# WxuanYuan/diffusynth

Measured on AMD Instinct MI355X. Metric: denoising-steps/sec (batch x T) on 256x64 latents, higher is better.
Workload: dtype bf16x3; 1 GPU; BASELINE configs[2]: DiffSynthSampler.sample() wall-clock, production ConditionedUnet (random init, torch.manual_seed(0)), bf16x3 (fp32 tensors, dense convolutions as 3 bf16 MFMA terms with fp32 accumulation: meets 1e-3 vs the fp32 reference), batch 64/GPU, latent (4,256,64), text condition, CFG=6.0 (U-Net batch 128 per step), 33-step respaced ddpm schedule, Philox noise on device; global_batch=64, parallelism=batch-shard x1, weights replicated

## Files before the change

### diffusynth_amd/csrc/dwconv_gn.hip

```cpp
#include <type_traits>

#include "common.hpp"

namespace {

constexpr int DW_TH = 4;
constexpr int DW_BLOCK = 256;

struct DwSrc { const char* base; int Cs, cc, Hs, Ws, oh, ow, buf; };
template <int ES>
__device__ __forceinline__ DwSrc dw_src(const ds_dwconv_params& p, int b, int c0) {
    if (c0 < p.C0) return {reinterpret_cast<const char*>(p.src0) + (size_t)b * p.H * p.W * p.C0 * ES, p.C0, c0, p.H, p.W, 0, 0, DS_BX_SRC0};
    return {reinterpret_cast<const char*>(p.src1) + (size_t)b * p.H1 * p.W1 * p.C1 * ES, p.C1, c0 - p.C0, p.H1, p.W1, p.off_h1, p.off_w1, DS_BX_SRC1};
}

template <int SR, int V, typename LoadRow>
__device__ __forceinline__ void dw_tap_column(float (&acc)[SR][V], const float* wcol, int pitch, LoadRow load_row) {
    float wv[7][V];
#pragma unroll
    for (int dh = 0; dh < 7; ++dh)
#pragma unroll
        for (int v = 0; v < V; v += 4) {
            const f32x4 t4 = *reinterpret_cast<const f32x4*>(wcol + dh * pitch + v);
            wv[dh][v] = t4[0]; wv[dh][v + 1] = t4[1]; wv[dh][v + 2] = t4[2]; wv[dh][v + 3] = t4[3];
        }
#pragma unroll
    for (int r = 0; r < SR + 6; ++r) {
        float x[V];
        load_row(r, x);
#pragma unroll
        for (int dh = 0; dh < 7; ++dh) {
            const int o = r - dh;
            if (o >= 0 && o < SR) {
#pragma unroll
                for (int v = 0; v < V; ++v) acc[o][v] = fmaf(x[v], wv[dh][v], acc[o][v]);
            }
        }
    }
}

template <typename T>
__device__ __forceinline__ float2 dw_store_row(const ds_dwconv_params& p, bool split, int b, int h, int w, int C, int c, const float* a, float2 s) {
    if (split) {
        bf16* o2 = reinterpret_cast<bf16*>(p.out) + ((size_t)b * p.H * p.W + (size_t)(h * p.W + w)) * (2 * C) + c;
        uint2 hi, lo;
        ds_split2(a[0], a[1], hi.x, lo.x);
        ds_split2(a[2], a[3], hi.y, lo.y);
        DS_ST(bf16x4, o2, DS_BX_OUT, __builtin_bit_cast(bf16x4, hi));
        DS_ST(bf16x4, o2 + C, DS_BX_OUT, __builtin_bit_cast(bf16x4, lo));
    } else {
        T* outp = reinterpret_cast<T*>(p.out) + (size_t)b * p.H * p.W * C;
        vec16_store<T>(outp + ((size_t)(h * p.W + w) * C + c), a, DS_BX_OUT);
    }
#pragma unroll
    for (int v = 0; v < Vec16<T>::N; ++v) {
        s.x += a[v];
        s.y += a[v] * a[v];
    }
    return s;
}

template <typename T>
__global__ __launch_bounds__(DW_BLOCK) void dwconv7_kernel(const ds_dwconv_params p, int nstrip, int CV) {
    constexpr int V = Vec16<T>::N;
    __shared__ float red[2 * (DW_BLOCK / 64)];
    const int C = p.C0 + p.C1;
    const int b = blockIdx.y;
    const long gid = (long)blockIdx.x * DW_BLOCK + threadIdx.x;
    const long total = (long)nstrip * p.W * CV;
    float2 st = {0.f, 0.f};
    if (gid < total) {
        const int cv = gid % CV;
        const int w = (gid / CV) % p.W;
        const int strip = gid / ((long)CV * p.W);
        const int h0 = strip * DW_TH;
        const int c = cv * V;
        const DwSrc s = dw_src<sizeof(T)>(p, b, c);
        const T* base = reinterpret_cast<const T*>(s.base);
        float acc[DW_TH][V];
        float init[V];
#pragma unroll
        for (int v = 0; v < V; ++v) {
            init[v] = p.bias[c + v];
            if (p.tbias) init[v] += p.tbias[(size_t)b * p.tb_stride + c + v];
        }
#pragma unroll
        for (int t = 0; t < DW_TH; ++t)
#pragma unroll
            for (int v = 0; v < V; ++v) acc[t][v] = init[v];

        for (int dw = 0; dw < 7; ++dw) {
            const int wi = w + dw - 3 - s.ow;
            if ((unsigned)wi >= (unsigned)s.Ws) continue;
            float col[DW_TH + 6][V];
#pragma unroll
            for (int r = 0; r < DW_TH + 6; ++r) {
                const int hi = h0 + r - 3 - s.oh;
                if ((unsigned)hi < (unsigned)s.Hs) {
                    vec16_load<T>(base + ((size_t)(hi * s.Ws + wi) * s.Cs + s.cc), col[r], s.buf);
                } else {
#pragma unroll
                    for (int v = 0; v < V; ++v) col[r][v] = 0.f;
                }
            }
#pragma unroll
            for (int dh = 0; dh < 7; ++dh) {
                float wv[V];
                const float* wp = p.wt + (size_t)(dh * 7 + dw) * C + c;
#pragma unroll
                for (int v = 0; v < V; v += 4) {
                    f32x4 t4 = DS_LD(f32x4, wp + v, DS_BX_W);
                    wv[v] = t4[0]; wv[v + 1] = t4[1]; wv[v + 2] = t4[2]; wv[v + 3] = t4[3];
                }
#pragma unroll
                for (int t = 0; t < DW_TH; ++t)
#pragma unroll
                    for (int v = 0; v < V; ++v) acc[t][v] = fmaf(col[t + dh][v], wv[v], acc[t][v]);
            }
        }
#pragma unroll
        for (int t = 0; t < DW_TH; ++t)
            if (h0 + t < p.H) st = dw_store_row<T>(p, false, b, h0 + t, w, C, c, acc[t], st);
    }
    if (p.stats_part) block_stats_write(st.x, st.y, red, p.stats_part + ((size_t)b * gridDim.x + blockIdx.x) * 2);
}

constexpr int LT_SR = 8;
constexpr int LT_NT = 2048 / LT_SR;
template <int TWL, int NV>
struct LT {
    static constexpr int W = 1 << TWL, H = (2048 / NV) >> TWL, HC = W + 6, HR = H + 6, NPX = HC * HR;
};
static int lt_twl(int W, int nv) { return W <= 8 ? 3 : ((W <= 16 || nv == 8) ? 4 : 5); }

template <typename T, int TWL, int LT_NV>
__global__ __launch_bounds__(LT_NT) void dwconv7_lds_kernel(const ds_dwconv_params p, int tiles_w, int tiles_hw, int ncblk) {
    constexpr int LT_W = LT<TWL, LT_NV>::W, LT_H = LT<TWL, LT_NV>::H, LT_HC = LT<TWL, LT_NV>::HC, LT_NPX = LT<TWL, LT_NV>::NPX;
    static_assert(LT_NV * LT_W * (LT_H / LT_SR) == LT_NT && LT_H % LT_SR == 0, "thread map");
    constexpr int V = Vec16<T>::N;
    constexpr int CB = LT_NV * V;
    extern __shared__ __attribute__((aligned(16))) char dsm[];
    uint4* xs = reinterpret_cast<uint4*>(dsm);
    float* wsm = reinterpret_cast<float*>(dsm + (size_t)LT_NPX * LT_NV * 16);
    float* red = wsm + 49 * CB;
    const int tid = threadIdx.x;
    const int wid = blockIdx.x + gridDim.x * blockIdx.y;
    const int cblk = wid % ncblk, tile = (wid / ncblk) % tiles_hw, b = wid / (tiles_hw * ncblk);
    const int bix = tile * ncblk + cblk;
    const int th = tile / tiles_w, tw = tile - th * tiles_w;
    const int h0 = th * LT_H, w0 = tw * LT_W, c0 = cblk * CB;
    const int C = p.C0 + p.C1;
    const DwSrc s = dw_src<sizeof(T)>(p, b, c0);
    const T* base = reinterpret_cast<const T*>(s.base);
#if DS_BOUNDS
    for (int slot = tid; slot < LT_NPX * LT_NV; slot += LT_NT) {
        const int px = slot / LT_NV, v = slot - px * LT_NV;
        const int hr = px / LT_HC, hc = px - hr * LT_HC;
        const int hi = h0 + hr - 3 - s.oh, wi = w0 + hc - 3 - s.ow;
        uint4 val = make_uint4(0, 0, 0, 0);
        if ((unsigned)hi < (unsigned)s.Hs && (unsigned)wi < (unsigned)s.Ws)
            val = DS_LD(uint4, base + ((size_t)(hi * s.Ws + wi) * s.Cs + s.cc + v * V), s.buf);
        xs[slot] = val;
    }
    for (int i = tid; i < 49 * CB; i += LT_NT) wsm[i] = DS_LD(float, p.wt + (size_t)(i / CB) * C + c0 + (i % CB), DS_BX_W);
#else
    {
        constexpr int SLOTS = LT_NPX * LT_NV, ITS = (SLOTS + LT_NT - 1) / LT_NT;
        const __amdgpu_buffer_rsrc_t rs = __builtin_amdgcn_make_buffer_rsrc(const_cast<T*>(base), (short)0, (int)((size_t)s.Hs * s.Ws * s.Cs * sizeof(T)), 0x00020000);
        const __amdgpu_buffer_rsrc_t rs_w = __builtin_amdgcn_make_buffer_rsrc(const_cast<float*>(p.wt), (short)0, 49 * C * 4, 0x00020000);
        u32x4 hv[ITS];
#pragma unroll
        for (int it = 0; it < ITS; ++it) {
            const int slot = tid + it * LT_NT;
            const int px = slot / LT_NV, v = slot - px * LT_NV;
            const int hr = px / LT_HC, hc = px - hr * LT_HC;
            const int hi = h0 + hr - 3 - s.oh, wi = w0 + hc - 3 - s.ow;
            const unsigned bad = (unsigned)(slot >= SLOTS) | (unsigned)((unsigned)hi >= (unsigned)s.Hs) | (unsigned)((unsigned)wi >= (unsigned)s.Ws);
            const unsigned off = (unsigned)((hi * s.Ws + wi) * s.Cs + s.cc + v * V) * (unsigned)sizeof(T);
            hv[it] = __builtin_amdgcn_raw_buffer_load_b128(rs, (int)((off & 0x7fffffffu) | (bad << 31)), 0, 0);
        }
        constexpr int WP = 49 * CB / 4, WIT = (WP + LT_NT - 1) / LT_NT;
        asm volatile("" : "+v"(hv[ITS - 1]));
        u32x4 wv4[WIT];
#pragma unroll
        for (int k = 0; k < WIT; ++k) {
            const int wp = tid + k * LT_NT, wtap = wp / (CB / 4), wj = wp - wtap * (CB / 4);
            wv4[k] = __builtin_amdgcn_raw_buffer_load_b128(rs_w, (int)((unsigned)((wtap * C + c0 + 4 * wj) * 4) | ((unsigned)(wp >= WP) << 31)), 0, 0);
        }
#pragma unroll
        for (int it = 0; it < ITS; ++it) {
            const int slot = tid + it * LT_NT;
            if (it + 1 < ITS || slot < SLOTS) *reinterpret_cast<u32x4*>(xs + slot) = hv[it];
        }
#pragma unroll
        for (int k = 0; k < WIT; ++k)
            if (tid + k * LT_NT < WP) *reinterpret_cast<u32x4*>(wsm + 4 * (tid + k * LT_NT)) = wv4[k];
    }
#endif
    const int cv = tid % LT_NV, wl = (tid / LT_NV) % LT_W, strip = tid / (LT_NV * LT_W);
    const int c = c0 + cv * V;
    float acc[LT_SR][V];
    {
        float init[V];
#if DS_BOUNDS
#pragma unroll
        for (int v = 0; v < V; ++v) {
            init[v] = p.bias[c + v];
            if (p.tbias) init[v] += p.tbias[(size_t)b * p.tb_stride + c + v];
        }
#else
        const __amdgpu_buffer_rsrc_t rs_b = __builtin_amdgcn_make_buffer_rsrc(const_cast<float*>(p.bias), (short)0, C * 4, 0x00020000);
        const __amdgpu_buffer_rsrc_t rs_t = __builtin_amdgcn_make_buffer_rsrc(const_cast<float*>(p.tbias ? p.tbias + (size_t)b * p.tb_stride : p.bias),
                                                                               (short)0, p.tbias ? C * 4 : 0, 0x00020000);
#pragma unroll
        for (int v = 0; v < V; v += 4) {
            const u32x4 b4 = __builtin_amdgcn_raw_buffer_load_b128(rs_b, (c + v) * 4, 0, 0), t4 = __builtin_amdgcn_raw_buffer_load_b128(rs_t, (c + v) * 4, 0, 0);
#pragma unroll
            for (int j = 0; j < 4; ++j) init[v + j] = __uint_as_float(b4[j]) + __uint_as_float(t4[j]);
        }
#endif
        __syncthreads();
#pragma unroll
        for (int o = 0; o < LT_SR; ++o)
#pragma unroll
            for (int v = 0; v < V; ++v) acc[o][v] = init[v];
    }
#pragma unroll 1
    for (int dw = 0; dw < 7; ++dw)
        dw_tap_column<LT_SR, V>(acc, wsm + dw * CB + cv * V, 7 * CB, [&](int r, float* x) {
            Vec16<T>::load(reinterpret_cast<const T*>(xs + ((strip * LT_SR + r) * LT_HC + wl + dw) * LT_NV + cv), x);
        });
    float2 st = {0.f, 0.f};
    const int w = w0 + wl;
#pragma unroll
    for (int o = 0; o < LT_SR; ++o) {
        const int h = h0 + strip * LT_SR + o;
        if (h < p.H && w < p.W) st = dw_store_row<T>(p, sizeof(T) == 4 && p.out_split, b, h, w, C, c, acc[o], st);
    }
    if (p.stats_part) block_stats_write(st.x, st.y, red, p.stats_part + ((size_t)b * gridDim.x + bix) * 2);
}

constexpr int ST_W = 16, ST_R = 16, ST_HC = ST_W + 6, ST_HR = ST_R + 6, ST_NT = 256;
constexpr int ST_ROWB = ST_HC * 8 * 16;
constexpr int ST_XS = ST_HR * ST_ROWB;
constexpr int ST_LDS = ST_XS + 49 * 32 * 4 + 64;

__global__ __launch_bounds__(ST_NT, 2) void dwconv7_strip_kernel(const ds_dwconv_params p, int strips_w, int ncblk, int hparts, int rows_per_part) {
    extern __shared__ __attribute__((aligned(16))) char dsm[];
    char* const xs = dsm;
    float* const wsm = reinterpret_cast<float*>(dsm + ST_XS);
    float* const red = wsm + 49 * 32;
    const int tid = threadIdx.x;
    const int nwg = gridDim.x;
    int wid = blockIdx.x;
    if ((nwg & 7) == 0) wid = (wid & 7) * (nwg >> 3) + (wid >> 3);
    const int cblk = wid % ncblk, sw = (wid / ncblk) % strips_w, hp = (wid / (strips_w * ncblk)) % hparts, b = wid / (strips_w * ncblk * hparts);
    const int bix = (hp * strips_w + sw) * ncblk + cblk;
    const int w0 = sw * ST_W, c0 = cblk * 32;
    const int hbeg = hp * rows_per_part, hend = min(p.H, hbeg + rows_per_part);
    const int ntile = (hend - hbeg + ST_R - 1) / ST_R;
    const int C = p.C0 + p.C1;
    const DwSrc s = dw_src<4>(p, b, c0);
    const int hc = tid >> 3, sv = tid & 7;
    const bool stager = hc < ST_HC;
    const int wi = w0 + hc - 3 - s.ow;
    const bool col_ok = stager && (unsigned)wi < (unsigned)s.Ws;
    const unsigned colbyte = (unsigned)((wi * s.Cs + s.cc + sv * 4) * 4);
    const unsigned rowpitch = (unsigned)(s.Ws * s.Cs * 4);
#if !DS_BOUNDS
    const __amdgpu_buffer_rsrc_t rs = __builtin_amdgcn_make_buffer_rsrc(const_cast<char*>(s.base), (short)0, (int)((size_t)s.Hs * s.Ws * s.Cs * 4), 0x00020000);
#endif
    auto load_rows = [&](u32x4* dst, int row0, auto nc) {
        constexpr int n = decltype(nc)::value;
#pragma unroll
        for (int it = 0; it < n; ++it) {
            const int hi = row0 + it - s.oh;
            const unsigned bad = (unsigned)(!col_ok) | (unsigned)((unsigned)hi >= (unsigned)s.Hs);
#if DS_BOUNDS
            dst[it] = u32x4{0u, 0u, 0u, 0u};
            if (!bad) dst[it] = DS_LD(u32x4, s.base + (size_t)hi * rowpitch + colbyte, s.buf);
#else
            const unsigned off = (unsigned)hi * rowpitch + colbyte;
            dst[it] = __builtin_amdgcn_raw_buffer_load_b128(rs, (int)((off & 0x7fffffffu) | (bad << 31)), 0, 0);
#endif
        }
    };
    auto store_rows = [&](const u32x4* src, int slot0, auto nc) {
        constexpr int n = decltype(nc)::value;
#pragma unroll
        for (int it = 0; it < n; ++it) {
            int sl = slot0 + it;
            sl = sl >= ST_HR ? sl - ST_HR : sl;
            *reinterpret_cast<u32x4*>(xs + sl * ST_ROWB + tid * 16) = src[it];
        }
    };
    auto lds_barrier = [&]() {
        asm volatile("s_waitcnt lgkmcnt(0)" ::: "memory");
        __builtin_amdgcn_s_barrier();
        asm volatile("" ::: "memory");
    };
    using N6 = std::integral_constant<int, 6>;
    using N16 = std::integral_constant<int, ST_R>;

    u32x4 hv[ST_R];
    u32x4 h6[6];
    if (stager) {
        load_rows(h6, hbeg - 3, N6{});
        load_rows(hv, hbeg + 3, N16{});
    }
    {
        constexpr int WP = 49 * 32 / 4, WIT = (WP + ST_NT - 1) / ST_NT;
#pragma unroll
        for (int k = 0; k < WIT; ++k) {
            const int wp = tid + k * ST_NT, wtap = wp >> 3, wj = wp & 7;
            if (wp < WP) *reinterpret_cast<f32x4*>(wsm + 4 * wp) = DS_LD(f32x4, p.wt + (size_t)wtap * C + c0 + 4 * wj, DS_BX_W);
        }
    }
    const int cv = tid & 7, wl = (tid >> 3) & 15, strip = tid >> 7;
    const int c = c0 + cv * 4;
    float init[4];
    {
        const f32x4 b4 = DS_LD(f32x4, p.bias + c, DS_BX_BIAS);
        f32x4 t4 = {0.f, 0.f, 0.f, 0.f};
        if (p.tbias) t4 = DS_LD(f32x4, p.tbias + (size_t)b * p.tb_stride + c, DS_BX_AUX1);
#pragma unroll
        for (int j = 0; j < 4; ++j) init[j] = b4[j] + t4[j];
    }
    if (stager) {
        store_rows(h6, 0, N6{});
        store_rows(hv, 6, N16{});
    }
    lds_barrier();

    float2 st = {0.f, 0.f};
    int rbase = 0;
    const int w = w0 + wl;
    const int colb = wl * 128 + cv * 16;
#pragma unroll 1
    for (int t = 0; t < ntile; ++t) {
        const int htop = hbeg + t * ST_R;
        const bool more = t + 1 < ntile;
        if (more && stager) load_rows(hv, htop + ST_R + 3, N16{});
        int roff[LT_SR + 6];
#pragma unroll
        for (int r = 0; r < LT_SR + 6; ++r) {
            int sl = rbase + strip * LT_SR + r;
            sl = sl >= ST_HR ? sl - ST_HR : sl;
            sl = sl >= ST_HR ? sl - ST_HR : sl;
            roff[r] = sl * ST_ROWB + colb;
        }
        float acc[LT_SR][4];
#pragma unroll
        for (int o = 0; o < LT_SR; ++o)
#pragma unroll
            for (int v = 0; v < 4; ++v) acc[o][v] = init[v];
#pragma unroll 1
        for (int dw = 0; dw < 7; ++dw)
            dw_tap_column<LT_SR, 4>(acc, wsm + dw * 32 + cv * 4, 7 * 32, [&](int r, float* x) {
                Vec16<float>::load(reinterpret_cast<const float*>(xs + roff[r] + dw * 128), x);
            });
        lds_barrier();
        if (more) {
            int ws = rbase + ST_R + 6;
            ws = ws >= ST_HR ? ws - ST_HR : ws;
            ws = ws >= ST_HR ? ws - ST_HR : ws;
            if (stager) store_rows(hv, ws, N16{});
            rbase = rbase + ST_R >= ST_HR ? rbase + ST_R - ST_HR : rbase + ST_R;
        }
#pragma unroll
        for (int o = 0; o < LT_SR; ++o) {
            const int h = htop + strip * LT_SR + o;
            if (h < hend && w < p.W) st = dw_store_row<float>(p, p.out_split, b, h, w, C, c, acc[o], st);
        }
        if (more) lds_barrier();
    }
    __syncthreads();
    if (p.stats_part) block_stats_write(st.x, st.y, red, p.stats_part + ((size_t)b * (hparts * strips_w * ncblk) + bix) * 2);
}

constexpr int MF_CB = 32;
template <bool TALL> struct M2 {
    static constexpr int W = TALL ? 16 : 32, H = TALL ? 32 : 16;
    static constexpr int HR = H + 6;
    static constexpr int HC = TALL ? 24 : 40;
    static constexpr int PLANE = HR * HC, SKEW = 32;
    static constexpr int BLK2 = TALL ? 16 * HC : 16;
    static constexpr int PBYTES = (MF_CB * PLANE + 3 * SKEW) * 2;
    static constexpr int OFF_O = 2 * PBYTES, OBYTES = H * W * MF_CB * 2, OFF_RED = OFF_O + OBYTES, LDS = OFF_RED + 64;
    static constexpr int SLOTS = HR * (HC / 4) * 4;
    static_assert(LDS <= 160 * 1024, "one block per CU");
};

struct Dw2Geo { int tiles_w, tiles, ncblk, tpc, nchunk, total; };
typedef __amdgpu_buffer_rsrc_t dw_rsrc_t;
__device__ __forceinline__ u32x4 dw_buf_ld16(dw_rsrc_t rs, const char* base, unsigned voff, int bounds_buf) {
#if DS_BOUNDS
    if (voff >= 0x80000000u || !ds_bx_ok(base + voff, bounds_buf, 16)) return u32x4{0u, 0u, 0u, 0u};
#endif
    (void)base; (void)bounds_buf;
    return __builtin_amdgcn_raw_buffer_load_b128(rs, (int)voff, 0, 0);
}

template <int NW, bool TALL>
__global__ __launch_bounds__(NW * 64, 1) void dwconv7_mfma2_kernel(const ds_dwconv_params p, const Dw2Geo g) {
    using G = M2<TALL>;
    constexpr int M2_W = G::W, M2_H = G::H, M2_HC = G::HC, M2_PLANE = G::PLANE, M2_SKEW = G::SKEW, M2_PBYTES = G::PBYTES, M2_OFF_O = G::OFF_O,
                  M2_OFF_RED = G::OFF_RED, M2_SLOTS = G::SLOTS;
    constexpr int NT = NW * 64, CPW = MF_CB / NW, SIT = (M2_SLOTS + NT - 1) / NT, OIT = M2_H * M2_W * 4 / NT;
    extern __shared__ __attribute__((aligned(16))) char dsm[];
    float* red = reinterpret_cast<float*>(dsm + M2_OFF_RED);
    const int tid = threadIdx.x, lane = tid & 63, wave = tid >> 6;
    const int NB = gridDim.x;
    int lid = blockIdx.x;
    if (NB % 8 == 0) lid = (blockIdx.x & 7) * (NB >> 3) + (blockIdx.x >> 3);
    if (lid >= g.total) return;
    const int nmy = (g.total - lid + NB - 1) / NB;
    const int nt = nmy * g.tpc - ((lid + (nmy - 1) * NB) / g.ncblk == g.nchunk - 1 ? g.nchunk * g.tpc - p.B * g.tiles : 0);
    const int C = p.C0 + p.C1;
    const bf16* wexp = reinterpret_cast<const bf16*>(p.wexp);

    struct Tile { dw_rsrc_t rs; int c, j, tile, th, tw, b, c0, h0, w0; DwSrc s; };
    auto set_sample = [&](Tile& t) {
        t.s = dw_src<2>(p, t.b, t.c0);
        t.rs = __builtin_amdgcn_make_buffer_rsrc(const_cast<char*>(t.s.base), (short)0, t.s.Hs * t.s.Ws * t.s.Cs * 2, 0x00020000);
    };
    auto start_chunk = [&](int c) {
        Tile t;
        t.c = c;
        t.j = 0;
        const int cblk = c % g.ncblk, item = (c / g.ncblk) * g.tpc;
        t.b = item / g.tiles;
        t.tile = item - t.b * g.tiles;
        t.th = t.tile / g.tiles_w;
        t.tw = t.tile - t.th * g.tiles_w;
        t.h0 = t.th * M2_H;
        t.w0 = t.tw * M2_W;
        t.c0 = cblk * MF_CB;
        set_sample(t);
        return t;
    };
    auto next_tile = [&](Tile t) {
        if (t.j + 1 == g.tpc) return start_chunk(t.c + NB);
        ++t.j;
        if (++t.tile == g.tiles) {
            t.tile = 0; t.th = 0; t.tw = 0;
            ++t.b;
            set_sample(t);
        } else if (++t.tw == g.tiles_w) { t.tw = 0; ++t.th; }
        t.h0 = t.th * M2_H;
        t.w0 = t.tw * M2_W;
        return t;
    };

    int s_hr[SIT], s_hc[SIT], s_lds[SIT];
    bool s_ok[SIT];
    const int sv = tid & 3;
#pragma unroll
    for (int it = 0; it < SIT; ++it) {
        const int slot = tid + it * NT, qd = slot >> 2;
        s_ok[it] = slot < M2_SLOTS;
        s_hr[it] = qd / (M2_HC / 4);
        s_hc[it] = (qd - s_hr[it] * (M2_HC / 4)) * 4;
        s_lds[it] = ((sv * 8) * M2_PLANE + sv * M2_SKEW + s_hr[it] * M2_HC + s_hc[it]) * 2;
    }
    u32x4 fv[SIT][4];
    auto issue_halo = [&](const Tile& t) {
#pragma unroll
        for (int it = 0; it < SIT; ++it) {
            const int hi = t.h0 + s_hr[it] - 3 - t.s.oh, wi = t.w0 + s_hc[it] - 3 - t.s.ow;
            const unsigned badr = (unsigned)(!s_ok[it]) | (unsigned)((unsigned)hi >= (unsigned)t.s.Hs);
            const unsigned o = (unsigned)((hi * t.s.Ws + wi) * t.s.Cs + t.s.cc + sv * 8) * 2u;
#pragma unroll
            for (int e = 0; e < 4; ++e) {
                const unsigned bad = badr | (unsigned)((unsigned)(wi + e) >= (unsigned)t.s.Ws);
                fv[it][e] = dw_buf_ld16(t.rs, t.s.base, ((o + (unsigned)(e * t.s.Cs) * 2u) & 0x0fffffffu) | (bad << 31), t.s.buf);
            }
        }
    };
    auto fill_planes = [&](char* pl) {
#pragma unroll
        for (int it = 0; it < SIT; ++it) {
            if (s_ok[it]) {
                char* dst = pl + s_lds[it];
#pragma unroll
                for (int j = 0; j < 4; ++j) {
                    const unsigned a = fv[it][0][j], b2 = fv[it][1][j], c2 = fv[it][2][j], d = fv[it][3][j];
                    typedef unsigned u32x2_t __attribute__((ext_vector_type(2)));
                    *reinterpret_cast<u32x2_t*>(dst + (2 * j) * (M2_PLANE * 2)) =
                        u32x2_t{__builtin_amdgcn_perm(b2, a, 0x05040100u), __builtin_amdgcn_perm(d, c2, 0x05040100u)};
                    *reinterpret_cast<u32x2_t*>(dst + (2 * j + 1) * (M2_PLANE * 2)) =
                        u32x2_t{__builtin_amdgcn_perm(b2, a, 0x07060302u), __builtin_amdgcn_perm(d, c2, 0x07060302u)};
                }
            }
        }
    };

    const int m = lane & 15, kq = lane >> 4;
    int aoff[6];
#pragma unroll
    for (int ks = 0; ks < 6; ++ks) {
        const int dh = 4 * (ks & 1) + kq, wg = ks >> 1;
        aoff[ks] = (m + (dh > 6 ? 6 : dh)) * M2_HC + 8 * wg;
    }
    bf16x8 wv[CPW][6];
    float addv[CPW];
    auto load_addv = [&](const Tile& t) {
        const int cb = t.c0 + wave * CPW;
#pragma unroll
        for (int k = 0; k < CPW; ++k) {
            addv[k] = DS_LD(float, p.bias + cb + k, DS_BX_BIAS);
            if (p.tbias) addv[k] += DS_LD(float, p.tbias + (size_t)t.b * p.tb_stride + cb + k, DS_BX_AUX1);
        }
    };
    auto load_chunk_consts = [&](const Tile& t) {
        const int cb = t.c0 + wave * CPW;
#pragma unroll
        for (int ci = 0; ci < CPW; ++ci) {
            const bf16* we = wexp + ((size_t)(cb + ci) * 6 * 64 + lane) * 8;
#pragma unroll
            for (int ks = 0; ks < 6; ++ks) wv[ci][ks] = DS_LD(bf16x8, we + ks * 64 * 8, DS_BX_AUX0);
        }
        load_addv(t);
    };

    Tile cur = start_chunk(lid);
    issue_halo(cur);
    load_chunk_consts(cur);
    fill_planes(dsm);
    __syncthreads();
    float s1 = 0.f, s2 = 0.f;
    char* const ot = dsm + M2_OFF_O;
    auto tile_body = [&](const int u, auto more_t) {
        constexpr bool more = decltype(more_t)::value;
        char* const pl = dsm + (u & 1) * M2_PBYTES;
        Tile nxt = cur;
        if constexpr (more) {
            nxt = next_tile(cur);
            issue_halo(nxt);
        }
        float outv[2][4][CPW];
#pragma unroll
        for (int ci = 0; ci < CPW; ++ci) {
            const int cl = wave * CPW + ci;
            const bf16* plane = reinterpret_cast<const bf16*>(pl) + cl * M2_PLANE + (cl >> 3) * M2_SKEW;
            f32x4 acc0 = {0.f, 0.f, 0.f, 0.f}, acc1 = {0.f, 0.f, 0.f, 0.f};
#pragma unroll
            for (int ks = 0; ks < 6; ++ks) {
                const bf16x8 a0 = *reinterpret_cast<const bf16x8*>(plane + aoff[ks]);
                const bf16x8 a1 = *reinterpret_cast<const bf16x8*>(plane + aoff[ks] + G::BLK2);
                acc0 = __builtin_amdgcn_mfma_f32_16x16x32_bf16(a0, wv[ci][ks], acc0, 0, 0, 0);
                acc1 = __builtin_amdgcn_mfma_f32_16x16x32_bf16(a1, wv[ci][ks], acc1, 0, 0, 0);
            }
#pragma unroll
            for (int r = 0; r < 4; ++r) {
                outv[0][r][ci] = acc0[r] + addv[ci];
                outv[1][r][ci] = acc1[r] + addv[ci];
            }
        }
#pragma unroll
        for (int wb = 0; wb < 2; ++wb)
#pragma unroll
            for (int r = 0; r < 4; ++r)
                if (cur.h0 + (TALL ? 16 * wb : 0) + kq * 4 + r < p.H && cur.w0 + (TALL ? 0 : 16 * wb) + m < p.W) {
#pragma unroll
                    for (int v = 0; v < CPW; ++v) {
                        s1 += outv[wb][r][v];
                        s2 = fmaf(outv[wb][r][v], outv[wb][r][v], s2);
                    }
                }
#pragma unroll
        for (int wb = 0; wb < 2; ++wb)
#pragma unroll
            for (int r = 0; r < 4; ++r) {
                typedef __bf16 bf16xc_t __attribute__((ext_vector_type(CPW)));
                bf16xc_t pk;
#pragma unroll
                for (int v = 0; v < CPW; ++v) pk[v] = (bf16)outv[wb][r][v];
                const int col = (TALL ? 0 : 16 * wb) + m, row = (TALL ? 16 * wb : 0) + kq * 4 + r, cbyte = wave * CPW * 2;
                *reinterpret_cast<bf16xc_t*>(ot + (row * M2_W + col) * 64 + (((cbyte >> 4) ^ ((col >> 1) & 3)) * 16) + (cbyte & 15)) = pk;
            }
        __syncthreads();
        const bool chunk_end = cur.j + 1 == g.tpc, sample_end = chunk_end || cur.tile + 1 == g.tiles;
        if (sample_end && p.stats_part) {
            const int nps = g.tiles >= g.tpc ? g.tiles / g.tpc : 1, kk = g.tiles >= g.tpc ? cur.tile / g.tpc : 0;
            block_stats_write(s1, s2, red, p.stats_part + ((size_t)cur.b * (nps * g.ncblk) + kk * g.ncblk + cur.c0 / MF_CB) * 2);
            s1 = 0.f;
            s2 = 0.f;
        }
        if constexpr (more) {
            if (chunk_end || sample_end) {
                if (chunk_end) load_chunk_consts(nxt);
                else load_addv(nxt);
#pragma unroll
                for (int ci = 0; ci < CPW; ++ci)
#pragma unroll
                    for (int ks = 0; ks < 6; ++ks) asm volatile("" : "+v"(wv[ci][ks]));
#pragma unroll
                for (int ci = 0; ci < CPW; ++ci) asm volatile("" : "+v"(addv[ci]));
            }
            fill_planes(dsm + ((u + 1) & 1) * M2_PBYTES);
        }
        {
            bf16* outp = reinterpret_cast<bf16*>(p.out) + (size_t)cur.b * p.H * p.W * C;
#pragma unroll
            for (int k = 0; k < OIT; ++k) {
                const int piece = tid + k * NT, px = piece >> 2, q = piece & 3;
                const int col = px % M2_W, h = cur.h0 + px / M2_W, w = cur.w0 + col;
                if (h < p.H && w < p.W) {
                    const u32x4 v = *reinterpret_cast<const u32x4*>(ot + px * 64 + ((q ^ ((col >> 1) & 3)) * 16));
                    DS_ST(u32x4, outp + ((size_t)(h * p.W + w) * C + cur.c0 + q * 8), DS_BX_OUT, v);
                }
            }
        }
        __syncthreads();
        cur = nxt;
    };
    for (int u = 0; u + 1 < nt; ++u) tile_body(u, std::true_type{});
    tile_body(nt - 1, std::false_type{});
}

static int dw_batch(const ds_dwconv_params* p) { return p->batch_hint > 0 ? p->batch_hint : p->B; }

static bool dw_tall(const ds_dwconv_params* p) { return p->W <= 16; }
static Dw2Geo dw2_geo(const ds_dwconv_params* p) {
    const int tw = dw_tall(p) ? 16 : 32, th = dw_tall(p) ? 32 : 16;
    Dw2Geo g;
    g.tiles_w = (p->W + tw - 1) / tw;
    g.tiles = g.tiles_w * ((p->H + th - 1) / th);
    g.ncblk = (p->C0 + p->C1) / MF_CB;
    g.tpc = 1;
    for (int d = 2; d <= 8; ++d)
        if ((g.tiles % d == 0 || (d % g.tiles == 0 && dw_batch(p) % (d / g.tiles) == 0 && g.ncblk <= 256)) && (long long)dw_batch(p) * g.tiles / d * g.ncblk >= 512) g.tpc = d;
    g.nchunk = (p->B * g.tiles + g.tpc - 1) / g.tpc;
    g.total = g.nchunk * g.ncblk;
    return g;
}

__global__ void pack_dw_mfma_kernel(const float* w, int C, bf16* dst) {
    const long i = (long)blockIdx.x * blockDim.x + threadIdx.x;
    if (i >= (long)C * 6 * 64 * 8) return;
    const int j = i & 7, lane = (i >> 3) & 63, ks = (i >> 9) % 6, c = i / (6 * 64 * 8);
    const int n = lane & 15, kq = lane >> 4;
    const int dh = 4 * (ks & 1) + kq, wg = ks >> 1, wp = 8 * wg + j, dw = wp - n;
    float v = 0.f;
    if (dh < 7 && dw >= 0 && dw < 7) v = w[(size_t)c * 49 + dh * 7 + dw];
    dst[i] = (bf16)v;
}

__global__ void pack_dw_kernel(const float* w, int C, float* dst) {
    const int i = blockIdx.x * blockDim.x + threadIdx.x;
    if (i < 49 * C) dst[i] = w[(size_t)(i % C) * 49 + i / C];
}

__global__ void gn_finalize_kernel(const float* part, int parts, double count, float eps, float* ab) {
    __shared__ double r1[256], r2[256];
    const int b = blockIdx.x;
    double a = 0.0, q = 0.0;
    for (int i = threadIdx.x; i < parts; i += blockDim.x) {
        a += (double)part[((size_t)b * parts + i) * 2];
        q += (double)part[((size_t)b * parts + i) * 2 + 1];
    }
    r1[threadIdx.x] = a;
    r2[threadIdx.x] = q;
// ... 601 lines not shown
```

Baseline: 721.8 denoising-steps/s.

## Software-pipeline depthwise 7x7 stencil with fully unrolled prefetched LDS loads

Replaces the per-column tap loop (runtime loop over dw, with weights loaded per column) with a fully unrolled 49-tap stencil that issues LDS weight and input-row loads a few taps ahead (DW_AHEAD=3). Scheduling barriers and empty asm constraints pin the ordering so the LDS load latency overlaps the FMAs. Input rows are loaded once per column as raw vectors and converted in place. This raises code size and register pressure, which could lower occupancy or cause spills under the kernel's launch bounds.

```diff
diff --git a/diffusynth_amd/csrc/dwconv_gn.hip b/diffusynth_amd/csrc/dwconv_gn.hip
--- a/diffusynth_amd/csrc/dwconv_gn.hip
+++ b/diffusynth_amd/csrc/dwconv_gn.hip
@@ -14,29 +14,60 @@
     return {reinterpret_cast<const char*>(p.src1) + (size_t)b * p.H1 * p.W1 * p.C1 * ES, p.C1, c0 - p.C0, p.H1, p.W1, p.off_h1, p.off_w1, DS_BX_SRC1};
 }
 
-template <int SR, int V, typename LoadRow>
-__device__ __forceinline__ void dw_tap_column(float (&acc)[SR][V], const float* wcol, int pitch, LoadRow load_row) {
-    float wv[7][V];
-#pragma unroll
-    for (int dh = 0; dh < 7; ++dh)
-#pragma unroll
-        for (int v = 0; v < V; v += 4) {
-            const f32x4 t4 = *reinterpret_cast<const f32x4*>(wcol + dh * pitch + v);
-            wv[dh][v] = t4[0]; wv[dh][v + 1] = t4[1]; wv[dh][v + 2] = t4[2]; wv[dh][v + 3] = t4[3];
-        }
-#pragma unroll
-    for (int r = 0; r < SR + 6; ++r) {
-        float x[V];
-        load_row(r, x);
-#pragma unroll
-        for (int dh = 0; dh < 7; ++dh) {
-            const int o = r - dh;
-            if (o >= 0 && o < SR) {
-#pragma unroll
-                for (int v = 0; v < V; ++v) acc[o][v] = fmaf(x[v], wv[dh][v], acc[o][v]);
-            }
-        }
-    }
+#ifndef DW_AHEAD
+#define DW_AHEAD 3
+#endif
+template <int G, int N, typename F>
+__device__ __forceinline__ void dw_static_for(F f) {
+    if constexpr (G < N) {
+        f(std::integral_constant<int, G>{});
+        dw_static_for<G + 1, N>(f);
+    }
+}
+template <typename T, int SR, int AHEAD, typename WAt, typename RowAt>
+__device__ __forceinline__ void dw_stencil(float (&acc)[SR][Vec16<T>::N], WAt w_at, RowAt row_at) {
+    constexpr int V = Vec16<T>::N;
+    f32x4 wr[49][V / 4];
+    u32x4 xr[7][SR + 6];
+    auto request = [&](auto gc) {
+        constexpr int g = decltype(gc)::value, dw = g / 7, dh = g % 7;
+#pragma unroll
+        for (int v = 0; v < V / 4; ++v) wr[g][v] = *reinterpret_cast<const f32x4*>(w_at(dw, dh) + 4 * v);
+#pragma unroll
+        for (int r = (dh ? dh + SR - 1 : 0); r < dh + SR; ++r) xr[dw][r] = *reinterpret_cast<const u32x4*>(row_at(dw, r));
+    };
+    dw_static_for<0, AHEAD>(request);
+    dw_static_for<0, 49>([&](auto gc) {
+        constexpr int g = decltype(gc)::value, dw = g / 7, dh = g % 7;
+        if constexpr (g + AHEAD < 49) request(std::integral_constant<int, g + AHEAD>{});
+        asm volatile("" : : : "memory");
+        __builtin_amdgcn_sched_barrier(0);
+#pragma unroll
+        for (int o = 0; o < SR; ++o) {
+            float x[V];
+            if constexpr (V == 4) {
+#pragma unroll
+                for (int v = 0; v < V; ++v) x[v] = __uint_as_float(xr[dw][o + dh][v]);
+            } else {
+                const bf16x8 b8 = __builtin_bit_cast(bf16x8, xr[dw][o + dh]);
+#pragma unroll
+                for (int v = 0; v < V; ++v) x[v] = (float)b8[v];
+            }
+#pragma unroll
+            for (int v = 0; v < V; ++v) acc[o][v] = fmaf(x[v], wr[g][v >> 2][v & 3], acc[o][v]);
+        }
+        if constexpr (g + 1 < 49) {
+#pragma unroll
+            for (int o = 0; o < SR; ++o)
+#pragma unroll
+                for (int v = 0; v < V; v += 4) {
+                    f32x4 a4 = {acc[o][v], acc[o][v + 1], acc[o][v + 2], acc[o][v + 3]};
+                    asm volatile("" : "+v"(a4) : : "memory");
+                    acc[o][v] = a4[0]; acc[o][v + 1] = a4[1]; acc[o][v + 2] = a4[2]; acc[o][v + 3] = a4[3];
+                }
+        }
+        __builtin_amdgcn_sched_barrier(0);
+    });
 }
 
 template <typename T>
@@ -225,11 +256,8 @@
 #pragma unroll
             for (int v = 0; v < V; ++v) acc[o][v] = init[v];
     }
-#pragma unroll 1
-    for (int dw = 0; dw < 7; ++dw)
-        dw_tap_column<LT_SR, V>(acc, wsm + dw * CB + cv * V, 7 * CB, [&](int r, float* x) {
-            Vec16<T>::load(reinterpret_cast<const T*>(xs + ((strip * LT_SR + r) * LT_HC + wl + dw) * LT_NV + cv), x);
-        });
+    dw_stencil<T, LT_SR, DW_AHEAD>(acc, [&](int dw, int dh) { return wsm + (dh * 7 + dw) * CB + cv * V; },
+                                   [&](int dw, int r) { return xs + ((strip * LT_SR + r) * LT_HC + wl + dw) * LT_NV + cv; });
     float2 st = {0.f, 0.f};
     const int w = w0 + wl;
 #pragma unroll
@@ -348,17 +376,15 @@
             sl = sl >= ST_HR ? sl - ST_HR : sl;
             sl = sl >= ST_HR ? sl - ST_HR : sl;
             roff[r] = sl * ST_ROWB + colb;
+            asm volatile("" : "+v"(roff[r]));
         }
         float acc[LT_SR][4];
 #pragma unroll
         for (int o = 0; o < LT_SR; ++o)
 #pragma unroll
             for (int v = 0; v < 4; ++v) acc[o][v] = init[v];
-#pragma unroll 1
-        for (int dw = 0; dw < 7; ++dw)
-            dw_tap_column<LT_SR, 4>(acc, wsm + dw * 32 + cv * 4, 7 * 32, [&](int r, float* x) {
-                Vec16<float>::load(reinterpret_cast<const float*>(xs + roff[r] + dw * 128), x);
-            });
+        dw_stencil<float, LT_SR, DW_AHEAD>(acc, [&](int dw, int dh) { return wsm + (dh * 7 + dw) * 32 + cv * 4; },
+                                           [&](int dw, int r) { return xs + roff[r] + dw * 128; });
         lds_barrier();
         if (more) {
             int ws = rbase + ST_R + 6;
```

Measured after the change: 722.4 denoising-steps/s, median of 6. No clear change (+0.1%).
